# eezkni/UEGAN

Hardware: AMD Instinct MI355X
Metric: train imgs/sec @512px bs=16 on 1/2/4/8 MI355X; infer ms/img (higher is better)
Workload: dtype bf16; 1 GPU; FiveK-shaped 512x512 batch=16/GPU, full G/D/VGG train step (trainer.py:77-119), conv_dim=32, seeded stand-in VGG19; global_batch=16, parallelism=dp1, pool_size=50, collective=none (1 rank), passes=batched (fused.py)

## Files before the change

include/uegan_hip.h:

```cpp
#ifndef UEGAN_HIP_H_
#define UEGAN_HIP_H_

#include <stddef.h>
#include <stdint.h>

#ifdef __cplusplus
extern "C" {
#endif

#define UEGAN_VERSION 105

enum { UEGAN_OK = 0, UEGAN_E_INVALID = -1, UEGAN_E_HIP = -2, UEGAN_E_UNSUPPORTED = -3 };
enum { UEGAN_F32 = 0, UEGAN_BF16 = 1 };
enum { UEGAN_PAD_ZERO = 0, UEGAN_PAD_REFLECT = 1 };
enum { UEGAN_ACT_NONE = 0, UEGAN_ACT_LRELU = 1, UEGAN_ACT_RELU = 2, UEGAN_ACT_TANH = 3,
       UEGAN_ACT_SIGMOID = 4,
       UEGAN_ACT_SWISH = 5, UEGAN_ACT_SELU = 6 };
enum { UEGAN_IMPL_AUTO = 0, UEGAN_IMPL_MFMA = 1, UEGAN_IMPL_DIRECT = 2, UEGAN_IMPL_MFMA_REGSTAGE = 3, UEGAN_IMPL_MFMA_GENERIC = 4 };

typedef void* uegan_stream_t;

int uegan_version(void);
const char* uegan_last_error(void);
int uegan_set_conv_impl(int impl);
enum {
  UEGAN_TUNE_SMALL_GRID = 0,
  UEGAN_TUNE_FOLD_MAX = 1,
  UEGAN_TUNE_HEADS_NO_CG = 2,
  UEGAN_TUNE_WIDE_MIN_GRID = 3,
  UEGAN_TUNE_TALL_MIN_GRID = 4,
  UEGAN_TUNE_TALL_RPW = 5,
  UEGAN_TUNE_TALL_REFLECT = 6,
  UEGAN_TUNE_FLAT_S2 = 7,
  UEGAN_TUNE_TOEP_HEADS = 8,
  UEGAN_TUNE_HEADS_MFMA = 9,
  UEGAN_TUNE_FWD_STATS = 10,
  UEGAN_TUNE_WGRAD_XCD = 11,
  UEGAN_TUNE_VGG_EPI = 12,
  UEGAN_TUNE_GAM_BWD = 13,
  UEGAN_TUNE_COUNT = 14
};
int uegan_set_tuning(int knob, int value, int* previous);
int uegan_selftest_mfma(void* scratch_4096_floats, uegan_stream_t stream);

typedef struct {
  char name[96];
  int64_t launches;
  double total_ms;
  double total_flops;
  double total_bytes;
} uegan_profile_entry;
int uegan_profile_begin(int max_records);
int uegan_profile_end(uegan_profile_entry* out, int max_entries, int* n_entries);

typedef struct {
// ... 23 lines not shown
  int64_t start;
  int32_t Cout, Cin, Cin_total, KH, KW, Cout_pad, Cin_pad, Kp, Kp2;
  int32_t flags;
  void* w_ohwi_lo;
} uegan_pack_entry;
int uegan_pack_weights_multi(int dtype, const uegan_pack_entry* table_dev, int n_entries, int64_t total, uegan_stream_t stream);
int uegan_conv2d_fwd(const uegan_conv_desc* d, const void* x1, const void* x2, const void* w_ohwi, const float* bias,
                     const float* scale, void* y, uegan_stream_t stream);
size_t uegan_conv2d_fwd_splitk_workspace_bytes(const uegan_conv_desc* d);
int uegan_conv2d_fwd_splitk(const uegan_conv_desc* d, const void* x1, const void* x2, const void* w_ohwi, const float* bias, const float* scale, void* y,
                            void* workspace, size_t workspace_bytes, uegan_stream_t stream);
size_t uegan_conv2d_fwd_stats_workspace_bytes(const uegan_conv_desc* d);
int uegan_conv2d_fwd_stats(const uegan_conv_desc* d, const void* x1, const void* x2, const void* w_ohwi, const float* bias, const float* scale, void* y,
                           float* mean, float* rstd, float eps, void* workspace, size_t workspace_bytes, int* produced, uegan_stream_t stream);
int uegan_instnorm_apply(int dtype, const void* x, void* y, const float* mean, const float* rstd, int B, int HW, int C, uegan_stream_t stream);

typedef struct {
  const void* x1_lo;
  const void* x2_lo;
  const void* w_lo;
  void* y_lo;
  const void* mul;
  const void* mul_lo;
  void* y_mul;
  void* y_mul_lo;
  const float* res_x;
  const float* res_x2;
  float* res_out;
  float* res_out2;
  float* mean;
// ... 231 lines not shown
```

uegan_amd/_lib.py:

```python
import ctypes as C
import os

_HERE = os.path.dirname(os.path.abspath(__file__))
LIB_PATH = os.path.join(_HERE, "libuegan_hip.so")
LIB_PATH_F16 = os.path.join(_HERE, "libuegan_hip_f16.so")

_lib = None
_lib_f16 = None
_use_f16 = False
_emulated = False

c_int, c_i64, c_f32, c_vp, c_sz = C.c_int, C.c_int64, C.c_float, C.c_void_p, C.c_size_t


class ConvDesc(C.Structure):
    _fields_ = [(n, C.c_int32) for n in ("dtype", "B", "H", "W", "C1", "C2", "Ho", "Wo", "Cout", "KH", "KW", "stride", "pad",
                                          "pad_mode", "act", "Cin_w", "Cout_w", "Cin_total", "scale_group")]


class ProfileEntry(C.Structure):
    _fields_ = [("name", C.c_char * 96), ("launches", c_i64), ("total_ms", C.c_double), ("total_flops", C.c_double),
                ("total_bytes", C.c_double)]


# ... 40 lines not shown
    "uegan_conv2d_fwd_splitk": (c_int, [C.POINTER(ConvDesc), c_vp, c_vp, c_vp, c_vp, c_vp, c_vp, c_vp, c_sz, c_vp]),
    "uegan_conv2d_fwd_pool": (c_int, [C.POINTER(ConvDesc), c_vp, c_vp, c_vp, c_vp, c_vp, c_vp, c_vp, c_vp]),
    "uegan_conv2d_fwd_pool_part": (c_int, [C.POINTER(ConvDesc), c_vp, c_vp, c_vp, c_vp, c_vp, c_vp, c_vp, c_int, c_vp]),
    "uegan_conv2d_fwd_pool_idx": (c_int, [C.POINTER(ConvDesc), c_vp, c_vp, c_vp, c_vp, c_vp, c_vp, c_vp, c_vp, c_int, c_int, c_vp]),
    "uegan_maxpool2x2_fwd_idx": (c_int, [c_int, c_vp, c_vp, c_vp, c_int, c_int, c_int, c_int, c_vp]),
    "uegan_maxpool2x2_bwd_idx": (c_int, [c_int, c_int, c_vp, c_vp, c_vp, c_vp, c_int, c_int, c_int, c_int, c_vp]),
    "uegan_conv2d_dgrad": (c_int, [C.POINTER(ConvDesc), c_vp, c_vp, c_vp, c_vp, c_vp, c_vp]),
    "uegan_conv2d_dgrad_workspace_bytes": (c_sz, [C.POINTER(ConvDesc)]),
    "uegan_conv2d_dgrad_ws": (c_int, [C.POINTER(ConvDesc), c_vp, c_vp, c_vp, c_vp, c_vp, c_vp, c_sz, c_vp]),
    "uegan_conv2d_dgrad_act": (c_int, [C.POINTER(ConvDesc), c_vp, c_vp, c_vp, c_vp, c_vp, c_sz, c_int, c_vp, c_vp]),
    "uegan_conv2d_dgrad_act_tap": (c_int, [C.POINTER(ConvDesc), c_vp, c_vp, c_vp, c_vp, c_int, c_vp, c_vp, c_f32, c_vp, c_vp, C.POINTER(c_int), c_vp]),
    "uegan_conv2d_dgrad_unpool": (c_int, [C.POINTER(ConvDesc), c_vp, c_vp, c_vp, c_vp, c_int, c_vp, c_vp, C.POINTER(c_int), c_vp]),
    "uegan_conv2d_fwd_stats_workspace_bytes": (c_sz, [C.POINTER(ConvDesc)]),
    "uegan_conv2d_fwd_stats": (c_int, [C.POINTER(ConvDesc), c_vp, c_vp, c_vp, c_vp, c_vp, c_vp, c_vp, c_vp, c_f32, c_vp, c_sz, C.POINTER(c_int), c_vp]),
    "uegan_instnorm_apply": (c_int, [c_int, c_vp, c_vp, c_vp, c_vp, c_int, c_int, c_int, c_vp]),
    "uegan_conv2d_dgrad_padded": (c_int, [C.POINTER(ConvDesc), c_vp, c_vp, c_vp, c_vp, c_vp, c_sz, C.POINTER(c_int), c_vp]),
    "uegan_conv2d_dgrad_padded_bytes": (c_sz, [C.POINTER(ConvDesc)]),
    "uegan_conv2d_wgrad_workspace_bytes": (c_sz, [C.POINTER(ConvDesc)]),
    "uegan_conv2d_wgrad": (c_int, [C.POINTER(ConvDesc), c_vp, c_vp, c_vp, c_vp, c_vp, c_vp, c_vp, c_sz, c_vp]),
    "uegan_conv2d_wgrad_acc": (c_int, [C.POINTER(ConvDesc), c_vp, c_vp, c_vp, c_vp, c_vp, c_vp, c_vp, c_sz, c_int, c_vp]),
    "uegan_act_bwd": (c_int, [c_int, c_int, c_vp, c_vp, c_vp, c_i64, c_vp]),
    "uegan_act_bwd2": (c_int, [c_int, c_int, c_vp, c_vp, c_vp, c_vp, c_i64, c_vp]),
    "uegan_act_bwd3": (c_int, [c_int, c_int, c_vp, c_vp, c_vp, c_vp, c_vp, c_i64, c_vp]),
    "uegan_nchw_to_nhwc": (c_int, [c_int, c_vp, c_vp, c_int, c_int, c_int, c_int, c_int, C.POINTER(c_f32), C.POINTER(c_f32), c_vp]),
    "uegan_nhwc_to_nchw": (c_int, [c_int, c_vp, c_vp, c_int, c_int, c_int, c_int, c_int, C.POINTER(c_f32), c_vp]),
    "uegan_residual_clamp_fwd": (c_int, [c_int, c_vp, c_vp, c_vp, c_int, c_int, c_int, c_int, c_int, c_vp]),
    "uegan_residual_clamp_bwd": (c_int, [c_int, c_vp, c_vp, c_vp, c_vp, c_vp, c_int, c_int, c_int, c_int, c_int, c_vp]),
    "uegan_residual_clamp_bwd_act": (c_int, [c_int, c_int, c_vp, c_vp, c_vp, c_vp, c_vp, c_int, c_int, c_int, c_int, c_int, c_vp]),
    "uegan_mul_bwd_act": (c_int, [c_int, c_int, c_int, c_vp, c_vp, c_vp, c_vp, c_vp, c_i64, c_vp]),
    "uegan_mul_fwd": (c_int, [c_int, c_vp, c_vp, c_vp, c_i64, c_vp]),
# ... 157 lines not shown
```

uegan_amd/csrc/conv.hip:

```cpp
#include "conv_stream.h"

namespace uegan {

int check_desc(const uegan_conv_desc* d) {
  UEGAN_CHECK_ARG(d != nullptr, "conv desc is null");
  UEGAN_CHECK_ARG(d->dtype == UEGAN_F32 || d->dtype == UEGAN_BF16, "bad dtype %d", d->dtype);
  UEGAN_CHECK_ARG(d->B > 0 && d->H > 0 && d->W > 0 && d->C1 > 0 && d->C2 >= 0 && d->Cout > 0, "bad conv dims");
  UEGAN_CHECK_ARG(d->KH > 0 && d->KW > 0 && d->stride > 0 && d->pad >= 0, "bad conv kernel/stride/pad");
  UEGAN_CHECK_ARG(d->Ho == (d->H + 2 * d->pad - d->KH) / d->stride + 1 && d->Wo == (d->W + 2 * d->pad - d->KW) / d->stride + 1,
                  "Ho/Wo inconsistent with H,W,pad,K,stride");
  if (d->pad_mode == UEGAN_PAD_REFLECT)
    UEGAN_CHECK_ARG(d->pad < d->H && d->pad < d->W, "reflection pad %d must be smaller than the input (%d x %d)", d->pad, d->H, d->W);
  else
    UEGAN_CHECK_ARG(d->pad_mode == UEGAN_PAD_ZERO, "bad pad mode");
  const int epc = d->dtype == UEGAN_F32 ? 4 : 8;
  UEGAN_CHECK_ARG(d->C1 % epc == 0 && d->C2 % epc == 0 && d->Cout % epc == 0,
                  "tensor channel counts must be multiples of %d (one 16-byte chunk): pad them (C1=%d C2=%d Cout=%d)", epc, d->C1, d->C2, d->Cout);
  UEGAN_CHECK_ARG(d->Cin_w >= 0 && d->Cin_w <= d->C1 + d->C2 && d->Cout_w >= 0 && d->Cout_w <= d->Cout, "bad true weight dims");
  UEGAN_CHECK_ARG(d->stride <= 2, "stride > 2 is not built");
  UEGAN_CHECK_ARG(d->scale_group >= 0, "bad scale_group");
  UEGAN_CHECK_ARG(d->Cin_total == 0 || d->Cin_total >= (d->Cin_w ? d->Cin_w : d->C1 + d->C2), "Cin_total must cover the input channels used");
  return UEGAN_OK;
}

// ... 204 lines not shown
  ConvArgs a;
  ConvStreamPlan sp;
  fwd_args(d, a, x1, x2, w_ohwi, bias, scale, y);
  if (!fwd_stats_plan(d, a, sp)) return uegan_conv2d_fwd(d, x1, x2, w_ohwi, bias, scale, y, stream);
  UEGAN_CHECK_ARG(mean && rstd && workspace && workspace_bytes >= uegan_conv2d_fwd_stats_workspace_bytes(d), "conv2d_fwd_stats: mean / rstd / workspace");
  hipStream_t s = (hipStream_t)stream;
  conv_stream_stats_arm(sp, workspace);
  {
    ProfScope prof = conv_stream_prof(sp, a.g.mode, s);
    conv_stream_launch(sp, s);
    UEGAN_CHECK_LAUNCH();
  }
  rc = conv_stream_stats_finalize(sp, mean, rstd, eps, s);
  if (rc == UEGAN_OK) *produced = 1;
  return rc;
}

static bool ex_plan(const uegan_conv_desc* d, const uegan_conv_ex* ex, ConvArgs& a, ConvStreamPlan& sp, bool* toep) {
  *toep = false;
  if (d->dtype != UEGAN_BF16 || g_impl.impl == UEGAN_IMPL_DIRECT || !g_impl.glds || !g_impl.stream || d->act > UEGAN_ACT_TANH) return false;
  a.in1_lo = ex->x1_lo; a.in2_lo = d->C2 ? ex->x2_lo : nullptr; a.w_lo = ex->w_lo; a.out_lo = ex->y_lo;
  a.mul = ex->mul; a.mul_lo = ex->mul_lo; a.out_mul = ex->y_mul; a.out_mul_lo = ex->y_mul_lo;
  a.res_x = ex->res_x; a.res_x2 = ex->res_x2; a.res_out = ex->res_out; a.res_out2 = ex->res_out2; a.res_split = ex->res_split > 0 ? ex->res_split : (1 << 30);
  if (ex->w_interleaved) {
    if (d->stride != 2 || d->C2 || (d->C1 != 32 && d->C1 != 64) || a.in1_lo || a.w_lo || a.out_lo || a.mul || a.res_out) return false;
    a.g.C = 2 * d->C1;
    a.src_wrap = d->C1 - 1;
    a.Kp = (int)uegan_packed_k((int64_t)d->KH * d->KW * a.g.C);
    *toep = false;
    return true;
// ... 259 lines not shown
```

uegan_amd/csrc/conv_core.h:

```cpp
#pragma once
#include "common.h"
#include "conv_internal.h"

#include <stdio.h>
#include <stdlib.h>
#include <utility>
#include <vector>

namespace uegan {

struct ProfRecord {
  hipEvent_t start, stop;
  int kernel_id;
  double flops, bytes;
};
extern bool g_prof_on;
extern std::vector<ProfRecord> g_prof_records;
extern std::vector<std::pair<hipEvent_t, hipEvent_t>> g_prof_pool;
extern size_t g_prof_used;

static inline int prof_key(int kind, bool bf16, int bn, int ks, int mode, int th, bool glds) {
  return (kind << 28) | ((bf16 ? 1 : 0) << 24) | (bn << 12) | (ks << 8) | (mode << 4) | ((th == 32 ? 2 : (th == 16 ? 1 : (th == 4 ? 3 : 0))) << 1) | (glds ? 1 : 0);
}
static const int PROF_PNG = 1 << 27;
// ... 201 lines not shown
  const float* epi_gscale = nullptr;
  float epi_weight = 0.f;
  const unsigned char* epi_idx = nullptr;
  int rect_y0 = 0, rect_y1 = 0, rect_x0 = 0, rect_x1 = 0;
  int border_only = 0;
  float* stats_part = nullptr;
  int stats_tpi = 0;
  const void* in1_lo = nullptr;
  const void* in2_lo = nullptr;
  const void* w_lo = nullptr;
  void* out_lo = nullptr;
  const void* mul = nullptr;
  const void* mul_lo = nullptr;
  void* out_mul = nullptr;
  void* out_mul_lo = nullptr;
  int src_wrap = 0;
  const float* res_x = nullptr;
  const float* res_x2 = nullptr;
  float* res_out = nullptr;
  float* res_out2 = nullptr;
  int res_split = 1 << 30;
  float* kws = nullptr;
  size_t kws_bytes = 0;
  int kparts = 0, kchunks = 0;
};

static inline int splitk_parts(const ConvArgs& a, int blocks, int nchunk, int* kchunks) {
  *kchunks = nchunk;
  if (!a.kws || a.g.mode != 0 || a.frame || a.out2 || a.mask || a.pool_out || a.stats_part || a.out_lo || a.mul || a.res_out || blocks <= 0) return 1;
  int parts = 1;
  while (parts * 2 <= nchunk && blocks * parts * 2 <= 256) parts *= 2;
  const size_t out_bytes = (size_t)a.g.B * a.g.OH * a.g.OW * a.N * sizeof(float);
  while (parts > 1 && (size_t)parts * out_bytes > a.kws_bytes) parts >>= 1;
  if (parts < 2) return 1;
  *kchunks = (nchunk + parts - 1) / parts;
  return (nchunk + *kchunks - 1) / *kchunks;
}

int splitk_reduce_launch(const ConvArgs& a, hipStream_t s);


constexpr int CONV_TH = 8, CONV_TW = 16, CONV_BM = CONV_TH * CONV_TW;
constexpr int CONV_ROWB = 128;

// ... 27 lines not shown
```

uegan_amd/csrc/conv_stream.h:

```cpp
#pragma once
#include "conv_core.h"

#include <type_traits>

namespace uegan {

struct ConvStreamArgs {
  ConvArgs c;
  int flip;
  int org;
  int zero_fill;
  int cls;
  int kstart[5];
  int ymin;
  int sx;
  int TH, PW, PH, PWmagic, KWmagic;
  int rb, rblog, Clog;
  int ksteps, taps;
  int wrow, wrows;
  int wbytes, tbytes, xbytes;
  int mtab_off;
  int xmir;
  int ty0, ty1, tx0, tx1;
  int tiles_total, tiles_per_block;
  int abl;
  int lo_xoff, c_lo, rb_lo, rblog_lo, wlo_off, tlo_off;
};

__device__ __forceinline__ int cs_swz(int rb, int pcol) {
  return rb == 128 ? swz128(pcol) : (rb == 64 ? swz64(pcol) : 0);
}

constexpr int CS_LDS_KB[4] = {53, 80, 152, 160};

template <int TN, int PF, int LC, bool CLS, bool XMIR = false, int NW = 4, bool STATS = false, int PR = 0, int EPX = 0>
__global__ void __launch_bounds__(64 * NW, (LC >= 2 ? 1 : (LC == 1 ? 2 : 3)) * NW / 4) conv_stream_kernel(ConvStreamArgs a) {
  constexpr int NT = 64 * NW;
  constexpr int MAXIX = (LC >= 2 ? 16 : 10) * 4 / NW;
  constexpr bool WLO = PR >= 1;
  static_assert(PR == 0 || (!CLS && !XMIR), "hi + lo pairs: plain forward only");
  __shared__ __attribute__((aligned(16))) unsigned char lds[CS_LDS_KB[LC] * 1024];
  const ConvArgs& ca = a.c;
  const ConvGeom& g = ca.g;
  const unsigned char* in1 = static_cast<const unsigned char*>(ca.in1);
  const unsigned char* in2 = static_cast<const unsigned char*>(ca.in2);
  const int tid = threadIdx.x, lane = tid & 63;
  const int wave = __builtin_amdgcn_readfirstlane(tid >> 6);
  const int fj = lane & 15, fg = lane >> 4;
  unsigned char* wl = lds;
  unsigned char* tab = lds + a.wbytes;
  unsigned char* xb0 = tab + a.tbytes;

  if (XMIR) {
    int* mflag = reinterpret_cast<int*>(tab + a.mtab_off) + 2 * a.ksteps * 64;
    for (int i = tid; i < 2 * a.ksteps; i += NT) mflag[i] = 0;
// ... 224 lines not shown
#pragma unroll
      for (int nf = 0; nf < TN; ++nf)
#pragma unroll
        for (int r = 0; r < 4; ++r) {
          float a1 = st1[nf][r], a2 = st2[nf][r];
#pragma unroll
          for (int o = 1; o < 16; o <<= 1) { a1 += __shfl_xor(a1, o, 64); a2 += __shfl_xor(a2, o, 64); }
          if (fj == 0) { dst[(nf * 16 + fg * 4 + r) * 2] = a1; dst[(nf * 16 + fg * 4 + r) * 2 + 1] = a2; }
          st1[nf][r] = 0.f; st2[nf][r] = 0.f;
        }
    }
  };
  const int row0 = wave * PF;
  int sc_grp = -1;
  float scale = 1.f;
  const int rowpitch = a.sx * a.PW * a.rb;
  for (int t = t_begin - 1; t < t_end; ++t) {
    const bool have = t >= t_begin;
    const int bufi = (t - t_begin) & 1;
    if (have) {
      wgtr_wait_loads();
      raw_barrier();
    }
    if (t + 1 < t_end && !((UEGAN_ABL_BITS(a.abl) & 1) && have)) stage(t + 1, bufi ^ 1);
    if (!have) continue;
    const unsigned char* xw = xb0 + bufi * a.xbytes + row0 * rowpitch;
    const int* tab2 = reinterpret_cast<const int*>(tab + a.ksteps * 256);
    constexpr int ncls = CLS ? 4 : 1;
   for (int cl = 0; cl < ncls; ++cl) {
    const int ks0 = CLS ? a.kstart[cl] : 0, ks1 = CLS ? a.kstart[cl + 1] : a.ksteps;
// ... 121 lines not shown
      }
    }
    int b, oy0, ox0;
    tile_origin(t, b, oy0, ox0);
    if (STATS && b != st_b) {
      if (st_b >= 0) stats_flush(st_b);
      st_b = b;
    }
    if (ca.scale) {
      const int grp = ca.scale_group ? b / ca.scale_group : 0;
      if (grp != sc_grp) {
        sc_grp = grp;
        scale = __builtin_bit_cast(float, __builtin_amdgcn_readfirstlane(__builtin_bit_cast(int, ca.scale[grp])));
      }
    }
    const int osx = CLS ? 2 : 1, opy = CLS ? (cl >> 1) : 0, opx = CLS ? (cl & 1) : 0;
    const int ox = osx * (ox0 + fj) + opx;
    const bool odd = fg & 1;
    auto epilogue = [&](auto act_c) {
      constexpr int ACT = decltype(act_c)::value;
#pragma unroll
      for (int i = 0; i < PF; ++i) {
        const int oy = osx * (oy0 + row0 + i) + opy;
        const bool pv = oy < g.OH && ox < g.OW;
        const size_t pixo = ((size_t)b * g.OH + oy) * g.OW + ox;
        uint32_t pk[TN][2];
        uint32_t pkl[EPX == 1 ? TN : 1][2], pkm[EPX == 2 ? TN : 1][2], pkml[EPX == 2 ? TN : 1][2];
#pragma unroll
        for (int nf = 0; nf < TN; ++nf) {
          float v[4];
#pragma unroll
          for (int r = 0; r < 4; ++r) v[r] = apply_act_c<ACT>(acc[nf][i][r] * scale + bv[nf][r]);
          if (STATS && pv) {
#pragma unroll
            for (int r = 0; r < 4; ++r) { st1[nf][r] += v[r]; st2[nf][r] += v[r] * v[r]; }
          }
          pk[nf][0] = pack_bf16x2(v[0], v[1]);
          pk[nf][1] = pack_bf16x2(v[2], v[3]);
          if constexpr (EPX != 0) {
            auto rest = [](float f, uint32_t packed, int hi) { return f - (hi ? half_hi_to_f32(packed) : half_lo_to_f32(packed)); };
            if constexpr (EPX == 1) {
              pkl[nf][0] = pack_bf16x2(rest(v[0], pk[nf][0], 0), rest(v[1], pk[nf][0], 1));
              pkl[nf][1] = pack_bf16x2(rest(v[2], pk[nf][1], 0), rest(v[3], pk[nf][1], 1));
            }
            if constexpr (EPX == 2) {
              const u32x2 mh = mulh[nf][i], ml = mull[nf][i];
              float q[4];
              q[0] = v[0] * (half_lo_to_f32(mh.x) + half_lo_to_f32(ml.x)); q[1] = v[1] * (half_hi_to_f32(mh.x) + half_hi_to_f32(ml.x));
              q[2] = v[2] * (half_lo_to_f32(mh.y) + half_lo_to_f32(ml.y)); q[3] = v[3] * (half_hi_to_f32(mh.y) + half_hi_to_f32(ml.y));
              pkm[nf][0] = pack_bf16x2(q[0], q[1]);
              pkm[nf][1] = pack_bf16x2(q[2], q[3]);
              if (ca.out_mul_lo) {
                pkml[nf][0] = pack_bf16x2(rest(q[0], pkm[nf][0], 0), rest(q[1], pkm[nf][0], 1));
                pkml[nf][1] = pack_bf16x2(rest(q[2], pkm[nf][1], 0), rest(q[3], pkm[nf][1], 1));
              }
            }
          }
        }
        if constexpr (EPX != 0) {
          auto emit = [&](const uint32_t (&k)[TN][2], void* dstp) {
#pragma unroll
            for (int pr = 0; pr < (TN + 1) / 2; ++pr) {
              const int nfa = 2 * pr, nfb = 2 * pr + 1 < TN ? 2 * pr + 1 : 2 * pr;
              const uint32_t s0 = odd ? k[nfa][0] : k[nfb][0], s1 = odd ? k[nfa][1] : k[nfb][1];
              const uint32_t r0 = __shfl_xor(s0, 16, 64), r1 = __shfl_xor(s1, 16, 64);
              const int nsel = odd ? nfb : nfa;
              const u32x4 chunk = odd ? u32x4{r0, r1, k[nfb][0], k[nfb][1]} : u32x4{k[nfa][0], k[nfa][1], r0, r1};
              const int n = nsel * 16 + (fg >> 1) * 8;
              if (!pv || n >= ca.N || (TN == 1 && odd)) continue;
              *reinterpret_cast<u32x4*>(static_cast<bf16_t*>(dstp) + pixo * ca.N + n) = chunk;
            }
          };
          emit(pk, ca.out);
// ... 34 lines not shown
      case UEGAN_ACT_TANH: epilogue(std::integral_constant<int, UEGAN_ACT_TANH>{}); break;
      default: epilogue(std::integral_constant<int, UEGAN_ACT_NONE>{}); break;
    }
   }
  }
  if (STATS && st_b >= 0) stats_flush(st_b);
}

struct ConvStreamPlan {
  ConvStreamArgs a;
  int tn, pf, blocks;
  int nw;
  int lc;
  bool fixup;
  bool stats = false;
  int pr = 0;
  int epx = 0;
};
bool conv_stream_launch_ex(const ConvStreamPlan& p, hipStream_t s);
bool conv_stream_ex_available(const ConvStreamPlan& p);

bool conv_stream_plan(const ConvArgs& c, int dtype, ConvStreamPlan& p, int max_pf = 4);
void conv_stream_launch(const ConvStreamPlan& p, hipStream_t s);
ProfScope conv_stream_prof(const ConvStreamPlan& p, int mode, hipStream_t s);
bool conv_stream_stats_ok(const ConvStreamPlan& p);
size_t conv_stream_stats_bytes(const ConvStreamPlan& p);
void conv_stream_stats_arm(ConvStreamPlan& p, void* workspace);
int conv_stream_stats_finalize(const ConvStreamPlan& p, float* mean, float* rstd, float eps, hipStream_t s);

}
// ... 1 lines not shown
```

uegan_amd/csrc/conv_stream.hip:

```cpp
#include "conv_stream.h"

namespace uegan {

bool conv_stream_plan(const ConvArgs& c, int dtype, ConvStreamPlan& p, int max_pf) {
  const ConvGeom& g = c.g;
  if (!g_impl.stream || dtype != UEGAN_BF16 || g.KH != g.KW || !(g.KH & 1) || g.pad != (g.KH - 1) / 2) return false;
  int pr = 0;
  if (c.w_lo) pr = (c.in1_lo && g.C2 == 0) ? 2 : ((c.in2_lo && !c.in1_lo && g.C1 == 32 && g.C2 == 32) ? 3 : ((c.in1_lo || c.in2_lo) ? -1 : 1));
  else if (c.in1_lo || c.in2_lo) pr = -1;
  const int epx = c.mul ? 2 : (c.out_lo ? 1 : 0);
  if (c.mul && c.out_lo) return false;
  if (pr >= 2 && !epx) return false;
  if (pr < 0 || ((pr || epx) && (g.mode != 0 || g.stride != 1 || c.mask || c.out2))) return false;
  if (pr >= 2 && g.pad_mode != UEGAN_PAD_REFLECT && g.pad != 0) return false;
  if (c.mul && !c.out_mul) return false;
  p.pr = pr; p.epx = epx;
  const int sx = g.stride;
  const bool cls = sx == 2 && g.mode == 1;
  if (cls) {
    if (!(g.C == 32 || g.C == 64) || g.OH != 2 * g.IH || g.OW != 2 * g.IW || g.pad_mode != UEGAN_PAD_REFLECT || g.C2 != 0) return false;
  } else if (sx == 2) {
    if (g.mode != 0 || g.OH != (g.IH + 2 * g.pad - g.KH) / 2 + 1 || g.OW != (g.IW + 2 * g.pad - g.KW) / 2 + 1) return false;
  } else if (sx != 1 || g.IH != g.OH || g.IW != g.OW) {
    return false;
  }
  if (!(g.C == 8 || g.C == 16 || g.C == 32 || g.C == 64) || c.N > 64 || c.N % 8 || (c.out2 && c.n_out1 % 8)) return false;
// ... 109 lines not shown
    }
    if (p.lc == 2) hipLaunchKernelGGL((conv_stream_kernel<TN, PF, 2, true>), dim3(blocks), dim3(256), 0, s, p.a);
    else hipLaunchKernelGGL((conv_stream_kernel<TN, PF, 1, true>), dim3(blocks), dim3(256), 0, s, p.a);
    return;
  }
  if constexpr (PF == 2 && TN <= 2) {
    if (p.nw == 8) {
      if (p.a.xmir) hipLaunchKernelGGL((conv_stream_kernel<TN, PF, 1, false, true, 8>), dim3(blocks), dim3(512), 0, s, p.a);
      else if (p.lc == 2) hipLaunchKernelGGL((conv_stream_kernel<TN, PF, 2, false, false, 8>), dim3(blocks), dim3(512), 0, s, p.a);
      else hipLaunchKernelGGL((conv_stream_kernel<TN, PF, 1, false, false, 8>), dim3(blocks), dim3(512), 0, s, p.a);
      return;
    }
  }
  if (p.stats) {
    if constexpr (TN >= 2) {
      hipLaunchKernelGGL((conv_stream_kernel<TN, PF, 1, false, false, 4, true>), dim3(blocks), dim3(256), 0, s, p.a);
      return;
    }
  }
  if (p.a.xmir) {
    if (p.lc == 2) hipLaunchKernelGGL((conv_stream_kernel<TN, PF, 2, false, true>), dim3(blocks), dim3(256), 0, s, p.a);
    else hipLaunchKernelGGL((conv_stream_kernel<TN, PF, 1, false, true>), dim3(blocks), dim3(256), 0, s, p.a);
    return;
  }
  if (p.lc == 2) hipLaunchKernelGGL((conv_stream_kernel<TN, PF, 2, false>), dim3(blocks), dim3(256), 0, s, p.a);
  else hipLaunchKernelGGL((conv_stream_kernel<TN, PF, 1, false>), dim3(blocks), dim3(256), 0, s, p.a);
}
bool conv_stream_stats_ok(const ConvStreamPlan& p) {
  const ConvGeom& g = p.a.c.g;
  const int tpi = (p.a.ty1 - p.a.ty0) * (p.a.tx1 - p.a.tx0);
  return g.mode == 0 && !p.a.cls && !p.a.xmir && p.nw == 4 && p.lc == 1 && !p.a.c.out2 && !p.a.c.mask && p.a.tiles_per_block <= tpi && p.tn >= 2;
// ... 198 lines not shown
```

uegan_amd/csrc/conv_stream_ex.hip:

```cpp
#include "conv_stream.h"

namespace uegan {

namespace {
struct ExKey { int tn, pf, lc, nw, stats, pr, epx; };
constexpr ExKey kEx[] = {
    {2, 2, 2, 8, 0, 0, 2},
    {2, 4, 1, 4, 0, 1, 1},
    {2, 4, 1, 4, 1, 2, 1},
    {2, 4, 1, 4, 0, 2, 1},
    {2, 2, 2, 8, 0, 2, 1},
    {2, 1, 2, 8, 0, 3, 2},
    {2, 4, 1, 4, 0, 1, 0},
};
int find(const ConvStreamPlan& p) {
  for (int i = 0; i < (int)(sizeof(kEx) / sizeof(kEx[0])); ++i) {
    const ExKey& k = kEx[i];
    if (k.tn == p.tn && k.pf == p.pf && k.lc == p.lc && k.nw == p.nw && k.stats == (p.stats ? 1 : 0) && k.pr == p.pr && k.epx == p.epx) return i;
  }
  return -1;
}
}

bool conv_stream_ex_available(const ConvStreamPlan& p) {
  if (p.a.cls || p.a.xmir) return false;
  ConvStreamPlan q = p;
  q.stats = false;
  if (find(q) >= 0) return true;
  q.stats = true;
  return find(q) >= 0;
}

bool conv_stream_launch_ex(const ConvStreamPlan& p, hipStream_t s) {
  const int blocks = p.blocks;
  switch (find(p)) {
    case 0: hipLaunchKernelGGL((conv_stream_kernel<2, 2, 2, false, false, 8, false, 0, 2>), dim3(blocks), dim3(512), 0, s, p.a); return true;
    case 1: hipLaunchKernelGGL((conv_stream_kernel<2, 4, 1, false, false, 4, false, 1, 1>), dim3(blocks), dim3(256), 0, s, p.a); return true;
    case 2: hipLaunchKernelGGL((conv_stream_kernel<2, 4, 1, false, false, 4, true, 2, 1>), dim3(blocks), dim3(256), 0, s, p.a); return true;
    case 3: hipLaunchKernelGGL((conv_stream_kernel<2, 4, 1, false, false, 4, false, 2, 1>), dim3(blocks), dim3(256), 0, s, p.a); return true;
    case 4: hipLaunchKernelGGL((conv_stream_kernel<2, 2, 2, false, false, 8, false, 2, 1>), dim3(blocks), dim3(512), 0, s, p.a); return true;
    case 5: hipLaunchKernelGGL((conv_stream_kernel<2, 1, 2, false, false, 8, false, 3, 2>), dim3(blocks), dim3(512), 0, s, p.a); return true;
    case 6: hipLaunchKernelGGL((conv_stream_kernel<2, 4, 1, false, false, 4, false, 1, 0>), dim3(blocks), dim3(256), 0, s, p.a); return true;
    default: return false;
  }
}

}
```

uegan_amd/csrc/runtime.hip:

```cpp
#include "conv_core.h"

#include <stdarg.h>

namespace uegan {

static thread_local char g_err[512] = "";

void set_error(const char* fmt, ...) {
  va_list ap;
  va_start(ap, fmt);
  vsnprintf(g_err, sizeof(g_err), fmt, ap);
  va_end(ap);
}

ConvImpl g_impl = {UEGAN_IMPL_AUTO, true, true, true, true, true};
int g_tuning[UEGAN_TUNE_COUNT] = {256, -1, 0, 192, 192, 0, 1, 1, 1, 1, 1, 1, 1, 1};
int g_abl_stream = 0, g_abl_wide = 0;
#ifdef UEGAN_TOOLS_BUILD
extern "C" int uegan_tools_set_ablation(int stream_wgrad_bits, int wide_variant) {
  g_abl_stream = stream_wgrad_bits;
  g_abl_wide = wide_variant;
  return UEGAN_OK;
}
#endif

bool g_prof_on = false;
std::vector<ProfRecord> g_prof_records;
std::vector<std::pair<hipEvent_t, hipEvent_t>> g_prof_pool;
size_t g_prof_used = 0;

__global__ void selftest_mfma_kernel(float* out) {
// ... 113 lines not shown
```

uegan_amd/models.py:

```python
import math


def _refuse_replica(m):
    if getattr(m, "_is_replica", False):
        raise RuntimeError("uegan_amd modules do not run as nn.DataParallel replicas (several device ids): use one process per GPU and "
                           "uegan_amd.trainer.Trainer -- see INTEGRATION.md")


import torch
import torch.nn as nn
import torch.nn.functional as F

from . import ops
from . import variants


def _require(cond, what):
    if not cond:
        raise NotImplementedError("uegan_amd implements the reference's default configuration only: " + what)


class ReflectionPadTag(nn.Module):

    def __init__(self, padding):
# ... 157 lines not shown

class GAM(nn.Module):

    def __init__(self, in_nc, out_nc, reduction=8, bias=False, use_sn=False, norm=False):
        super().__init__()
        _require(norm and not bias and in_nc == out_nc, "GAM(norm=True, bias=False)")
        self.conv = nn.Sequential(Conv2d(in_nc * 2, in_nc // reduction, 1, 1, bias=False), Identity(),
                                  Conv2d(in_nc // reduction, out_nc, 1, 1, bias=False))
        self.fuse = nn.Sequential((SpectralNormConv2d if use_sn else Conv2d)(in_nc * 2, out_nc, 1, 1, bias=True))
        self.use_sn = use_sn
        self.in_nc = in_nc
        self.norm = norm
        self._cfg = ops.ConvCfg(1, ops.PAD_REFLECT, ops.ACT_NONE, cin_used=in_nc)

    def forward(self, x, x_lo=None, pre=None):
        if pre is not None:
            z = self.fuse_in(x, x_lo)
            if x_lo is not None:
                y, y_lo = ops.instnorm_pair(z[0], z[1], pre)
            else:
                y = ops.instnorm(z, pre)
            y = self._touch(y)
            return y if x_lo is None else (y, y_lo)
        fuse = self.fuse[0]
        sn = ops.specnorm_sigma(fuse.weight_orig, fuse.weight_u, fuse.weight_v, do_iter=self.training) if self.use_sn else None
        holder = ops.StatsHolder()
        if x_lo is not None:
            ex = ops.ConvExtras(x1_lo=x_lo, pair_w=True, want_lo=True)
            y = ops.conv2d(x, None, fuse.weight, None, self._cfg, sn=sn, stats=holder, ex=ex)
            if holder.value is None:
# ... 269 lines not shown
```

uegan_amd/ops.py:

```python
import ctypes as C
import weakref

import torch

from . import _lib as L

ACT_NONE, ACT_LRELU, ACT_RELU, ACT_TANH = 0, 1, 2, 3
PAD_ZERO, PAD_REFLECT = 0, 1
IN_EPS = 1e-5
SN_EPS = 1e-12

_compute_dtype = torch.float32
_weight_epoch = [0]


def set_compute_dtype(dt):
    global _compute_dtype
    if dt not in (torch.float32, torch.bfloat16, torch.float16):
        raise ValueError("compute dtype must be float32, bfloat16 or float16")
    if dt != torch.float32:
        L.use_half_format("fp16" if dt == torch.float16 else "bf16")
    _compute_dtype = dt


# ... 570 lines not shown
        L.check(lib().uegan_instnorm_bwd(_dt(y), _p(g), _p(y), _p(stats[1]), _p(dx), _p(tmp), B, H * W, Cc, _stream()))
        return dx, None, None, None


def gam_bwd_ws_bytes(dtype, B, HW, Cc, x_act):
    if dtype == torch.float32:
        return 0
    return lib().uegan_gam_bwd_ws_bytes(1, B, HW, Cc, x_act)


class _GamHub(torch.autograd.Function):

    @staticmethod
    def forward(ctx, x, weight, cfg, x_act, n_x, wsb):
        x = x.contiguous()
        holder = StatsHolder()
        z, d, ihwo = raw_conv_fwd(x, None, weight, None, cfg, stats=holder)
        y = torch.empty_like(z)
        stats = _instnorm_into(z, y, holder.value)
        ctx.cfg, ctx.d, ctx.ihwo, ctx.pack_version = cfg, d, ihwo, cfg.packed.version
        ctx.x_act, ctx.wsb, ctx.wsink = x_act, wsb, _sink_of(weight)
        ctx.save_for_backward(x, y, stats, weight)
        return tuple(x.view_as(x) for _ in range(n_x)) + (y,)

    @staticmethod
    def backward(ctx, *gs):
        x, y, stats, weight = ctx.saved_tensors
        cfg, d = ctx.cfg, ctx.d
        gy = gs[-1]
        adds = [g.contiguous() for g in gs[:-1] if g is not None]
        if gy is None or len(adds) > 2:
            raise RuntimeError("gam_hub backward: the attention output's gradient and at most two further gradients of x expected")
        if cfg.packed.ihwo is ctx.ihwo and cfg.packed.version != ctx.pack_version:
            raise RuntimeError("gam_hub backward: the module's weight was updated by an optimizer step after this forward; run backward() before step()")
# ... 199 lines not shown
        L.check(lib().uegan_conv2d_fwd_pool_part(C.byref(d), _p(x1), _p(x2), _p(ohwi), _p(biasc), _p(scale), _p(y), _p(yp), nf, _stream()))
        return y, d, ihwo, yp
    wsb = lib().uegan_conv2d_fwd_stats_workspace_bytes(C.byref(d)) if stats is not None else 0
    if wsb:
        st = torch.empty((2, d.B, d.Cout), dtype=torch.float32, device=x1.device)
        ws = torch.empty(((wsb + 3) // 4,), dtype=torch.float32, device=x1.device)
        produced = C.c_int(0)
        L.check(lib().uegan_conv2d_fwd_stats(C.byref(d), _p(x1), _p(x2), _p(ohwi), _p(biasc), _p(scale), _p(y), _p(st[0]), _p(st[1]), IN_EPS, _p(ws), wsb,
                                             C.byref(produced), _stream()))
        stats.value = st if produced.value else None
        return y, d, ihwo
    if stats is not None:
        stats.value = None
    _fwd_plain(d, x1, x2, ohwi, biasc, scale, y)
    return y, d, ihwo


def raw_conv_dgrad(d, dz, ihwo, scale=None, in_act=ACT_NONE, x_act=None, nb=None, two=False):
    d = _sub_desc(d, nb)
    dev = dz.device
    dx1 = torch.empty((d.B, d.H, d.W, d.C1), dtype=dz.dtype, device=dev)
    dx2 = torch.empty((d.B, d.H, d.W, d.C2), dtype=dz.dtype, device=dev) if two else None
    dwsb = lib().uegan_conv2d_dgrad_workspace_bytes(C.byref(d))
    dws = torch.empty((dwsb + 3) // 4, dtype=torch.float32, device=dev) if dwsb else None
    st = _stream()
    if in_act != ACT_NONE:
        if two:
            raise RuntimeError("conv: in_act (deferred activation gradient) needs a single-input conv")
        L.check(lib().uegan_conv2d_dgrad_act(C.byref(d), _p(dz), _p(ihwo), _p(scale), _p(dx1), _p(dws), dwsb, in_act, _p(x_act), st))
    else:
# ... 414 lines not shown
```

Before: 515.0 imgs/sec.

## Fuse 1x1 conv with instance norm via a stats-only pass and a normalizing epilogue

Adds a conv+instnorm forward path for 1x1 stride-1 single-input convs. A first launch of the conv computes only the per-channel moments and stores nothing. A second launch recomputes the conv and applies (z-mean)*rstd in its epilogue. This removes the full write and re-read of the unnormalized intermediate and the separate instnorm_apply kernel, at the cost of running the GEMM twice. It is wired into the GAM hub forward and into a no-grad path of a model block, with an option to pass in precomputed moments.

```diff
diff --git a/include/uegan_hip.h b/include/uegan_hip.h
--- a/include/uegan_hip.h
+++ b/include/uegan_hip.h
@@ -38,7 +38,8 @@
   UEGAN_TUNE_WGRAD_XCD = 11,
   UEGAN_TUNE_VGG_EPI = 12,
   UEGAN_TUNE_GAM_BWD = 13,
-  UEGAN_TUNE_COUNT = 14
+  UEGAN_TUNE_FWD_NORM = 14,
+  UEGAN_TUNE_COUNT = 15
 };
 int uegan_set_tuning(int knob, int value, int* previous);
 int uegan_selftest_mfma(void* scratch_4096_floats, uegan_stream_t stream);
@@ -92,6 +93,9 @@
 int uegan_conv2d_fwd_stats(const uegan_conv_desc* d, const void* x1, const void* x2, const void* w_ohwi, const float* bias, const float* scale, void* y,
                            float* mean, float* rstd, float eps, void* workspace, size_t workspace_bytes, int* produced, uegan_stream_t stream);
 int uegan_instnorm_apply(int dtype, const void* x, void* y, const float* mean, const float* rstd, int B, int HW, int C, uegan_stream_t stream);
+size_t uegan_conv2d_fwd_norm_workspace_bytes(const uegan_conv_desc* d);
+int uegan_conv2d_fwd_norm(const uegan_conv_desc* d, const void* x1, const void* w_ohwi, const float* bias, const float* scale, void* y, float* mean,
+                          float* rstd, float eps, int given, void* workspace, size_t workspace_bytes, int* produced, uegan_stream_t stream);
 
 typedef struct {
   const void* x1_lo;
diff --git a/uegan_amd/_lib.py b/uegan_amd/_lib.py
--- a/uegan_amd/_lib.py
+++ b/uegan_amd/_lib.py
@@ -78,6 +78,8 @@
     "uegan_conv2d_fwd_stats_workspace_bytes": (c_sz, [C.POINTER(ConvDesc)]),
     "uegan_conv2d_fwd_stats": (c_int, [C.POINTER(ConvDesc), c_vp, c_vp, c_vp, c_vp, c_vp, c_vp, c_vp, c_vp, c_f32, c_vp, c_sz, C.POINTER(c_int), c_vp]),
     "uegan_instnorm_apply": (c_int, [c_int, c_vp, c_vp, c_vp, c_vp, c_int, c_int, c_int, c_vp]),
+    "uegan_conv2d_fwd_norm_workspace_bytes": (c_sz, [C.POINTER(ConvDesc)]),
+    "uegan_conv2d_fwd_norm": (c_int, [C.POINTER(ConvDesc), c_vp, c_vp, c_vp, c_vp, c_vp, c_vp, c_vp, c_f32, c_int, c_vp, c_sz, C.POINTER(c_int), c_vp]),
     "uegan_conv2d_dgrad_padded": (c_int, [C.POINTER(ConvDesc), c_vp, c_vp, c_vp, c_vp, c_vp, c_sz, C.POINTER(c_int), c_vp]),
     "uegan_conv2d_dgrad_padded_bytes": (c_sz, [C.POINTER(ConvDesc)]),
     "uegan_conv2d_wgrad_workspace_bytes": (c_sz, [C.POINTER(ConvDesc)]),
diff --git a/uegan_amd/csrc/conv.hip b/uegan_amd/csrc/conv.hip
--- a/uegan_amd/csrc/conv.hip
+++ b/uegan_amd/csrc/conv.hip
@@ -242,6 +242,54 @@
   rc = conv_stream_stats_finalize(sp, mean, rstd, eps, s);
   if (rc == UEGAN_OK) *produced = 1;
   return rc;
+}
+
+static bool fwd_norm_plan(const uegan_conv_desc* d, ConvArgs& a, ConvStreamPlan& sp1, ConvStreamPlan& sp2, const float* mean, const float* rstd) {
+  if (g_tuning[UEGAN_TUNE_FWD_NORM] == 0 || d->KH != 1 || d->KW != 1 || d->C2 != 0 || d->stride != 1) return false;
+  if (!fwd_stats_plan(d, a, sp1)) return false;
+  ConvArgs a2 = a;
+  a2.norm_mean = mean; a2.norm_rstd = rstd;
+  return conv_stream_plan(a2, d->dtype, sp2, a.N > 32 ? 2 : 4);
+}
+extern "C" size_t uegan_conv2d_fwd_norm_workspace_bytes(const uegan_conv_desc* d) {
+  if (check_desc(d)) return 0;
+  ConvArgs a;
+  ConvStreamPlan sp1, sp2;
+  static const float probe = 0.f;
+  fwd_args(d, a, nullptr, nullptr, nullptr, nullptr, nullptr, nullptr);
+  return fwd_norm_plan(d, a, sp1, sp2, &probe, &probe) ? conv_stream_stats_bytes(sp1) : 0;
+}
+extern "C" int uegan_conv2d_fwd_norm(const uegan_conv_desc* d, const void* x1, const void* w_ohwi, const float* bias, const float* scale, void* y,
+                                     float* mean, float* rstd, float eps, int given, void* workspace, size_t workspace_bytes, int* produced,
+                                     uegan_stream_t stream) {
+  int rc = check_desc(d);
+  if (rc) return rc;
+  UEGAN_CHECK_ARG(x1 && w_ohwi && y && mean && rstd && produced, "null pointer");
+  *produced = 0;
+  ConvArgs a;
+  ConvStreamPlan sp1, sp2;
+  fwd_args(d, a, x1, nullptr, w_ohwi, bias, scale, y);
+  if (!fwd_norm_plan(d, a, sp1, sp2, mean, rstd)) return UEGAN_OK;
+  hipStream_t s = (hipStream_t)stream;
+  if (!given) {
+    UEGAN_CHECK_ARG(workspace && workspace_bytes >= conv_stream_stats_bytes(sp1), "conv2d_fwd_norm: workspace");
+    conv_stream_stats_arm(sp1, workspace);
+    sp1.nost = true;
+    {
+      ProfScope prof = conv_stream_prof(sp1, a.g.mode, s);
+      conv_stream_launch(sp1, s);
+      UEGAN_CHECK_LAUNCH();
+    }
+    rc = conv_stream_stats_finalize(sp1, mean, rstd, eps, s);
+    if (rc) return rc;
+  }
+  {
+    ProfScope prof = conv_stream_prof(sp2, a.g.mode, s);
+    conv_stream_launch(sp2, s);
+    UEGAN_CHECK_LAUNCH();
+  }
+  *produced = 1;
+  return UEGAN_OK;
 }
 
 static bool ex_plan(const uegan_conv_desc* d, const uegan_conv_ex* ex, ConvArgs& a, ConvStreamPlan& sp, bool* toep) {
diff --git a/uegan_amd/csrc/conv_core.h b/uegan_amd/csrc/conv_core.h
--- a/uegan_amd/csrc/conv_core.h
+++ b/uegan_amd/csrc/conv_core.h
@@ -239,6 +239,8 @@
   const void* mul_lo = nullptr;
   void* out_mul = nullptr;
   void* out_mul_lo = nullptr;
+  const float* norm_mean = nullptr;
+  const float* norm_rstd = nullptr;
   int src_wrap = 0;
   const float* res_x = nullptr;
   const float* res_x2 = nullptr;
@@ -252,7 +254,7 @@
 
 static inline int splitk_parts(const ConvArgs& a, int blocks, int nchunk, int* kchunks) {
   *kchunks = nchunk;
-  if (!a.kws || a.g.mode != 0 || a.frame || a.out2 || a.mask || a.pool_out || a.stats_part || a.out_lo || a.mul || a.res_out || blocks <= 0) return 1;
+  if (!a.kws || a.g.mode != 0 || a.frame || a.out2 || a.mask || a.pool_out || a.stats_part || a.out_lo || a.mul || a.norm_mean || a.res_out || blocks <= 0) return 1;
   int parts = 1;
   while (parts * 2 <= nchunk && blocks * parts * 2 <= 256) parts *= 2;
   const size_t out_bytes = (size_t)a.g.B * a.g.OH * a.g.OW * a.N * sizeof(float);
diff --git a/uegan_amd/csrc/conv_stream.h b/uegan_amd/csrc/conv_stream.h
--- a/uegan_amd/csrc/conv_stream.h
+++ b/uegan_amd/csrc/conv_stream.h
@@ -33,12 +33,13 @@
 
 constexpr int CS_LDS_KB[4] = {53, 80, 152, 160};
 
-template <int TN, int PF, int LC, bool CLS, bool XMIR = false, int NW = 4, bool STATS = false, int PR = 0, int EPX = 0>
+template <int TN, int PF, int LC, bool CLS, bool XMIR = false, int NW = 4, bool STATS = false, int PR = 0, int EPX = 0, bool NOST = false>
 __global__ void __launch_bounds__(64 * NW, (LC >= 2 ? 1 : (LC == 1 ? 2 : 3)) * NW / 4) conv_stream_kernel(ConvStreamArgs a) {
   constexpr int NT = 64 * NW;
   constexpr int MAXIX = (LC >= 2 ? 16 : 10) * 4 / NW;
   constexpr bool WLO = PR >= 1;
   static_assert(PR == 0 || (!CLS && !XMIR), "hi + lo pairs: plain forward only");
+  static_assert(!NOST || (STATS && EPX == 0 && PR == 0), "a launch without stores exists for the moments alone");
   __shared__ __attribute__((aligned(16))) unsigned char lds[CS_LDS_KB[LC] * 1024];
   const ConvArgs& ca = a.c;
   const ConvGeom& g = ca.g;
@@ -293,6 +294,8 @@
   const int row0 = wave * PF;
   int sc_grp = -1;
   float scale = 1.f;
+  int nm_b = -1;
+  float nmean[EPX == 3 ? TN : 1][4], nrstd[EPX == 3 ? TN : 1][4];
   const int rowpitch = a.sx * a.PW * a.rb;
   for (int t = t_begin - 1; t < t_end; ++t) {
     const bool have = t >= t_begin;
@@ -444,6 +447,19 @@
         scale = __builtin_bit_cast(float, __builtin_amdgcn_readfirstlane(__builtin_bit_cast(int, ca.scale[grp])));
       }
     }
+    if constexpr (EPX == 3) {
+      if (b != nm_b) {
+        nm_b = b;
+#pragma unroll
+        for (int nf = 0; nf < TN; ++nf)
+#pragma unroll
+          for (int r = 0; r < 4; ++r) {
+            const int n = nf * 16 + fg * 4 + r;
+            nmean[nf][r] = n < ca.N ? ca.norm_mean[(size_t)b * ca.N + n] : 0.f;
+            nrstd[nf][r] = n < ca.N ? ca.norm_rstd[(size_t)b * ca.N + n] : 0.f;
+          }
+      }
+    }
     const int osx = CLS ? 2 : 1, opy = CLS ? (cl >> 1) : 0, opx = CLS ? (cl & 1) : 0;
     const int ox = osx * (ox0 + fj) + opx;
     const bool odd = fg & 1;
@@ -467,7 +483,10 @@
           }
           pk[nf][0] = pack_bf16x2(v[0], v[1]);
           pk[nf][1] = pack_bf16x2(v[2], v[3]);
-          if constexpr (EPX != 0) {
+          if constexpr (EPX == 3) {
+            pk[nf][0] = pack_bf16x2((half_lo_to_f32(pk[nf][0]) - nmean[nf][0]) * nrstd[nf][0], (half_hi_to_f32(pk[nf][0]) - nmean[nf][1]) * nrstd[nf][1]);
+            pk[nf][1] = pack_bf16x2((half_lo_to_f32(pk[nf][1]) - nmean[nf][2]) * nrstd[nf][2], (half_hi_to_f32(pk[nf][1]) - nmean[nf][3]) * nrstd[nf][3]);
+          } else if constexpr (EPX != 0) {
             auto rest = [](float f, uint32_t packed, int hi) { return f - (hi ? half_hi_to_f32(packed) : half_lo_to_f32(packed)); };
             if constexpr (EPX == 1) {
               pkl[nf][0] = pack_bf16x2(rest(v[0], pk[nf][0], 0), rest(v[1], pk[nf][0], 1));
@@ -487,6 +506,7 @@
             }
           }
         }
+        if constexpr (NOST) continue;
         if constexpr (EPX != 0) {
           auto emit = [&](const uint32_t (&k)[TN][2], void* dstp) {
 #pragma unroll
@@ -551,6 +571,7 @@
   int lc;
   bool fixup;
   bool stats = false;
+  bool nost = false;
   int pr = 0;
   int epx = 0;
 };
diff --git a/uegan_amd/csrc/conv_stream.hip b/uegan_amd/csrc/conv_stream.hip
--- a/uegan_amd/csrc/conv_stream.hip
+++ b/uegan_amd/csrc/conv_stream.hip
@@ -8,8 +8,8 @@
   int pr = 0;
   if (c.w_lo) pr = (c.in1_lo && g.C2 == 0) ? 2 : ((c.in2_lo && !c.in1_lo && g.C1 == 32 && g.C2 == 32) ? 3 : ((c.in1_lo || c.in2_lo) ? -1 : 1));
   else if (c.in1_lo || c.in2_lo) pr = -1;
-  const int epx = c.mul ? 2 : (c.out_lo ? 1 : 0);
-  if (c.mul && c.out_lo) return false;
+  const int epx = c.mul ? 2 : (c.out_lo ? 1 : (c.norm_mean ? 3 : 0));
+  if ((c.mul && c.out_lo) || (c.norm_mean && (c.mul || c.out_lo || pr || !c.norm_rstd))) return false;
   if (pr >= 2 && !epx) return false;
   if (pr < 0 || ((pr || epx) && (g.mode != 0 || g.stride != 1 || c.mask || c.out2))) return false;
   if (pr >= 2 && g.pad_mode != UEGAN_PAD_REFLECT && g.pad != 0) return false;
@@ -149,7 +149,8 @@
   }
   if (p.stats) {
     if constexpr (TN >= 2) {
-      hipLaunchKernelGGL((conv_stream_kernel<TN, PF, 1, false, false, 4, true>), dim3(blocks), dim3(256), 0, s, p.a);
+      if (p.nost) hipLaunchKernelGGL((conv_stream_kernel<TN, PF, 1, false, false, 4, true, 0, 0, true>), dim3(blocks), dim3(256), 0, s, p.a);
+      else hipLaunchKernelGGL((conv_stream_kernel<TN, PF, 1, false, false, 4, true>), dim3(blocks), dim3(256), 0, s, p.a);
       return;
     }
   }
diff --git a/uegan_amd/csrc/conv_stream_ex.hip b/uegan_amd/csrc/conv_stream_ex.hip
--- a/uegan_amd/csrc/conv_stream_ex.hip
+++ b/uegan_amd/csrc/conv_stream_ex.hip
@@ -12,6 +12,8 @@
     {2, 2, 2, 8, 0, 2, 1},
     {2, 1, 2, 8, 0, 3, 2},
     {2, 4, 1, 4, 0, 1, 0},
+    {2, 4, 1, 4, 0, 0, 3},
+    {4, 2, 1, 4, 0, 0, 3},
 };
 int find(const ConvStreamPlan& p) {
   for (int i = 0; i < (int)(sizeof(kEx) / sizeof(kEx[0])); ++i) {
@@ -41,6 +43,8 @@
     case 4: hipLaunchKernelGGL((conv_stream_kernel<2, 2, 2, false, false, 8, false, 2, 1>), dim3(blocks), dim3(512), 0, s, p.a); return true;
     case 5: hipLaunchKernelGGL((conv_stream_kernel<2, 1, 2, false, false, 8, false, 3, 2>), dim3(blocks), dim3(512), 0, s, p.a); return true;
     case 6: hipLaunchKernelGGL((conv_stream_kernel<2, 4, 1, false, false, 4, false, 1, 0>), dim3(blocks), dim3(256), 0, s, p.a); return true;
+    case 7: hipLaunchKernelGGL((conv_stream_kernel<2, 4, 1, false, false, 4, false, 0, 3>), dim3(blocks), dim3(256), 0, s, p.a); return true;
+    case 8: hipLaunchKernelGGL((conv_stream_kernel<4, 2, 1, false, false, 4, false, 0, 3>), dim3(blocks), dim3(256), 0, s, p.a); return true;
     default: return false;
   }
 }
diff --git a/uegan_amd/csrc/runtime.hip b/uegan_amd/csrc/runtime.hip
--- a/uegan_amd/csrc/runtime.hip
+++ b/uegan_amd/csrc/runtime.hip
@@ -14,7 +14,7 @@
 }
 
 ConvImpl g_impl = {UEGAN_IMPL_AUTO, true, true, true, true, true};
-int g_tuning[UEGAN_TUNE_COUNT] = {256, -1, 0, 192, 192, 0, 1, 1, 1, 1, 1, 1, 1, 1};
+int g_tuning[UEGAN_TUNE_COUNT] = {256, -1, 0, 192, 192, 0, 1, 1, 1, 1, 1, 1, 1, 1, 1};
 int g_abl_stream = 0, g_abl_wide = 0;
 #ifdef UEGAN_TOOLS_BUILD
 extern "C" int uegan_tools_set_ablation(int stream_wgrad_bits, int wide_variant) {
diff --git a/uegan_amd/models.py b/uegan_amd/models.py
--- a/uegan_amd/models.py
+++ b/uegan_amd/models.py
@@ -195,6 +195,10 @@
         self._cfg = ops.ConvCfg(1, ops.PAD_REFLECT, ops.ACT_NONE, cin_used=in_nc)
 
     def forward(self, x, x_lo=None, pre=None):
+        if x_lo is None and not self.use_sn and not torch.is_grad_enabled():
+            fused = ops.raw_conv_norm_fwd(x.contiguous(), self.fuse[0].weight, self._cfg, pre=pre)
+            if fused is not None:
+                return fused[0]
         if pre is not None:
             z = self.fuse_in(x, x_lo)
             if x_lo is not None:
diff --git a/uegan_amd/ops.py b/uegan_amd/ops.py
--- a/uegan_amd/ops.py
+++ b/uegan_amd/ops.py
@@ -608,10 +608,14 @@
     @staticmethod
     def forward(ctx, x, weight, cfg, x_act, n_x, wsb):
         x = x.contiguous()
-        holder = StatsHolder()
-        z, d, ihwo = raw_conv_fwd(x, None, weight, None, cfg, stats=holder)
-        y = torch.empty_like(z)
-        stats = _instnorm_into(z, y, holder.value)
+        fused = raw_conv_norm_fwd(x, weight, cfg)
+        if fused is not None:
+            y, stats, d, ihwo = fused
+        else:
+            holder = StatsHolder()
+            z, d, ihwo = raw_conv_fwd(x, None, weight, None, cfg, stats=holder)
+            y = torch.empty_like(z)
+            stats = _instnorm_into(z, y, holder.value)
         ctx.cfg, ctx.d, ctx.ihwo, ctx.pack_version = cfg, d, ihwo, cfg.packed.version
         ctx.x_act, ctx.wsb, ctx.wsink = x_act, wsb, _sink_of(weight)
         ctx.save_for_backward(x, y, stats, weight)
@@ -841,6 +845,28 @@
         stats.value = None
     _fwd_plain(d, x1, x2, ohwi, biasc, scale, y)
     return y, d, ihwo
+
+
+def raw_conv_norm_fwd(x, weight, cfg, scale=None, wkey=None, pre=None):
+    if x.dtype == torch.float32:
+        return None
+    d = _desc(x, None, weight, cfg)
+    wsb = lib().uegan_conv2d_fwd_norm_workspace_bytes(C.byref(d))
+    if not wsb:
+        return None
+    ohwi, ihwo = cfg.packed.get(weight, x.dtype, d.C1 + d.C2, d.Cout, wkey, cfg.cin_used)
+    y = torch.empty((d.B, d.Ho, d.Wo, d.Cout), dtype=x.dtype, device=x.device)
+    st = pre.contiguous() if pre is not None else torch.empty((2, d.B, d.Cout), dtype=torch.float32, device=x.device)
+    if st.dtype != torch.float32 or tuple(st.shape) != (2, d.B, d.Cout):
+        raise ValueError("conv + norm: float32 [2, %d, %d] moments expected" % (d.B, d.Cout))
+    ws = None if pre is not None else torch.empty(((wsb + 3) // 4,), dtype=torch.float32, device=x.device)
+    _chk(x, y, st)
+    produced = C.c_int(0)
+    L.check(lib().uegan_conv2d_fwd_norm(C.byref(d), _p(x), _p(ohwi), None, _p(scale), _p(y), _p(st[0]), _p(st[1]), IN_EPS, 0 if pre is None else 1,
+                                        _p(ws), wsb if pre is None else 0, C.byref(produced), _stream()))
+    if not produced.value:
+        raise RuntimeError("uegan_conv2d_fwd_norm declined a layer its size query had accepted")
+    return y, st, d, ihwo
 
 
 def raw_conv_dgrad(d, dz, ihwo, scale=None, in_act=ACT_NONE, x_act=None, nb=None, two=False):
```

After: 515.3 imgs/sec (median of 6 runs). Within noise of the previous version (+0.1%).
